# safijari/yag-slam

Hardware: AMD Instinct MI355X
Metric: pose hypotheses/sec (higher is better)
Workload: dtype u8

## Files before the change

yag_slam_amd/csrc/ym_abi_debug.hpp:

```cpp
int ym_debug_grid_info(ym_matcher *m, int item, ym_grid_info *info) {
    if (!m || !info) return set_err(YM_ERR_INVALID, "null argument");
    if (!m->last_valid || item < 0 || item >= m->last_B) return set_err(YM_ERR_INVALID, "no such item in the last call");
    const YmGeom &g = m->last_geom;
    info->width = g.win_w; info->height = g.win_w; info->pitch = g.pitch;
    info->origin_x = g.win_origin; info->origin_y = g.win_origin;
    info->storage_w = g.storage_w; info->storage_h = g.storage_w;
    info->roi_x = g.border; info->roi_y = g.border; info->roi_w = g.roi_w; info->roi_h = g.roi_w;
    YmItemState s;
    DEV_GUARD(m->device);
    HIP_TRY(hipStreamSynchronize(m->stream));
    HIP_TRY(hipMemcpy(&s, m->states.p + item, sizeof s, hipMemcpyDeviceToHost));
    info->offset_x = s.off_x; info->offset_y = s.off_y;
    return YM_OK;
}

int ym_debug_grid(ym_matcher *m, int item, uint8_t *out, int64_t out_bytes) {
    if (!m || !out) return set_err(YM_ERR_INVALID, "null argument");
    if (!m->last_valid || item < 0 || item >= m->last_B) return set_err(YM_ERR_INVALID, "no such item in the last call");
    const int64_t need = (int64_t)m->last_geom.pitch * m->last_geom.win_w;
    if (out_bytes < need) return set_err(YM_ERR_INVALID, "grid buffer too small: need %lld bytes", (long long)need);
    DEV_GUARD(m->device);
    HIP_TRY(hipStreamSynchronize(m->stream));
    HIP_TRY(hipMemcpy(out, m->grid.p + (size_t)item * m->last_grid_stride, (size_t)need, hipMemcpyDeviceToHost));
    return YM_OK;
// ... 24 lines not shown
    *n = s.nq;
    if (cap < s.nq) return set_err(YM_ERR_INVALID, "buffer too small: need %d points", s.nq);
    if (s.nq > 0)
        HIP_TRY(hipMemcpy(out_xy, s.ql, sizeof(double2) * s.nq, hipMemcpyDeviceToHost));
    return YM_OK;
}

int ym_debug_cells(ym_matcher *m, int item, int32_t *out, int64_t out_count, int32_t *max_n) {
    if (!m || !max_n) return set_err(YM_ERR_INVALID, "null argument");
    if (!m->last_valid || item < 0 || item >= m->last_B) return set_err(YM_ERR_INVALID, "no such item in the last call");
    *max_n = m->last_max_n;
    const size_t per = (size_t)m->last_max_base * m->last_max_n;
    if (!out) return YM_OK;
    if ((size_t)out_count < per * 2) return set_err(YM_ERR_INVALID, "buffer too small: need %zu ints", per * 2);
    DEV_GUARD(m->device);
    HIP_TRY(hipStreamSynchronize(m->stream));
    HIP_TRY(hipMemcpy(out, m->cells.p + (size_t)item * per, sizeof(int2) * per, hipMemcpyDeviceToHost));
    return YM_OK;
}

int ym_debug_option(ym_matcher *m, int option, int value) {
    if (m) { m->cache_gen++; m->list_key_valid = false; }
    if (!m) return set_err(YM_ERR_INVALID, "null matcher");
    if (option == 0) return set_err(YM_ERR_INVALID, "debug option 0 (an experimental correlate form) no longer exists");
    else if (option == 2) m->full_raster = value;
    else if (option == 3) m->corr_u = value;
    else if (option == 4) m->corr_pad_lds = value;
    else if (option == 5) m->corr_chunks = value;
    else if (option == 6) m->finish_form = value;
    else if (option == 9) m->corr_cw = value;
    else if (option == 10) m->select_global = value;
    else if (option == 41) m->select_split_max = value;
    else if (option == 11) m->finish_threads = value;
    else if (option == 12) m->keep_sums = value;
    else if (option == 13) m->corr_dedup = value;
    else if (option == 14) m->corr_region = value;
    else if (option == 15) m->corr_region_na = m->corr_region_nw = value;
    else if (option == 23) m->poll_completion = value != 0;
    else if (option == 24) m->use_scan_structure = value != 0;
    else if (option == 25) m->chain_margin = value;
    else if (option == 26) m->prepare_threads = value;
    else if (option == 28) {
        if (value == 0) { m->lds_min_batch = 64; m->rg_min_batch = 48; }
        else m->lds_min_batch = m->rg_min_batch = std::max(8, value);
    }
    else if (option == 42) m->rg_min_batch = value == 0 ? 48 : std::max(8, value);
    else if (option == 29) m->overlap_lists = value != 0;
    else if (option == 31) m->staged_queries = value != 0;
    else if (option == 30) m->tile_h_forced = value == YM_TILE_H || value == YM_TILE_H_TALL ? value : 0;
    else if (option == 16) m->raster_gx = value;
    else if (option == 17) m->corr_region_parts = value;
    else if (option == 21) m->corr_fuse_score = value;
    else if (option == 45) { m->list_cache_on = value != 0; m->list_key_valid = false; }
    else if (option == 46) m->yag_fast = value < 0 ? 0 : value > 2 ? 1 : value;
    else if (option == 43) m->rg2_h = value;
    else if (option == 44) {
#ifndef YM_EXPERIMENTAL
        return set_err(YM_ERR_UNSUPPORTED, "correlate_region2_kernel is compiled only into builds made with -DYM_EXPERIMENTAL");
#endif
        m->rg2_min_batch = value > 0 ? value : 1 << 30;
    }
    else if (option == 32) {
#ifndef YM_EXPERIMENTAL
        if (value >= 2) return set_err(YM_ERR_UNSUPPORTED, "correlate form %d is compiled only into builds made with -DYM_EXPERIMENTAL", value);
#endif
        m->corr_region_form = value;
    }
    else if (option == 33) m->corr_region_dbg = value;
    else if (option == 34) m->corr_region_rsplit = value;
    else if (option == 35) {
#ifndef YM_EXPERIMENTAL
        return set_err(YM_ERR_UNSUPPORTED, "correlate_item_kernel is compiled only into builds made with -DYM_EXPERIMENTAL");
#endif
        m->item_min_batch = value;
    }
    else if (option == 36) m->raster_planes_only = value;
    else if (option == 37) m->raster_no_rowtab = value;
    else if (option == 38) m->corr_region_pad_lds = value;
    else if (option == 39) m->keep_planes = value;
    else if (option == 40) m->tile_list_min_batch = value;
    else if (option == 19) m->corr_region_cap = value;
    else if (option == 20) m->corr_region_lds = value;
    else if (option == 18) m->raster_hits_per_tile = value;
    else if (option == 7) {
        m->cache_off = value == 1;
        m->cache_entries.clear();
        m->cache_index.clear();
        m->cache_used = 0;
    }
    else if (option == 8) {
        m->cache_limit = (size_t)std::max(1, value) << 10;
        HIP_TRY(hipStreamSynchronize(m->stream));
        m->cache_entries.clear();
        m->cache_index.clear();
        m->cache_used = 0;
        m->cache_arena.release();
    }
    else return set_err(YM_ERR_INVALID, "unknown option %d", option);
    return YM_OK;
}

int ym_debug_stamps(ym_matcher *m, int enable, uint64_t *out, int32_t count) {
    if (!m) return set_err(YM_ERR_INVALID, "null matcher");
    DEV_GUARD(m->device);
    HIP_TRY(hipStreamSynchronize(m->stream));
    if (out && count > 0)
// ... 54 lines not shown
```

yag_slam_amd/csrc/ym_host_enqueue.hpp:

```cpp
void enqueue_prepare(ym_matcher *m, const CallPlan &P) {
    ym::PrepareArgs a;
    a.scans = P.d_scans; a.items = P.d_items; a.g = P.g; a.lat = P.lc; a.states = m->states.p; a.qlocal = m->qlocal.p;
    a.cells = m->cells.p; a.bbox = m->bbox.p; a.ctrig = m->ctrig.p; a.hypcell = m->hypcell.p; a.probs = P.probs;
    a.max_n = P.max_n; a.max_base = P.max_base; a.nt_stride = P.nt_stride; a.dim_stride = P.dim_stride; a.stamps = P.stamps;
    a.use_inline = P.inline_desc ? 1 : 0;
    a.pad0 = 0;
    std::memset(&a.inl, 0, sizeof a.inl);
    if (a.use_inline) {
        a.inl.item = P.hi[0];
        for (int i = 0; i < P.nscans; i++) a.inl.scans[i] = P.hs[i];
    }
    a.qnp = m->qnp.p; a.jobs = P.d_jobs; a.job_slot = P.d_job_slot;
    a.fault = nullptr; a.step = 0; a.pad1 = 0;
    for (int k = 0; k < 4; k++) a.cell_box[k] = P.cell_box[k];
    if (P.chain_step) { a.fault = m->seq_fault.p; a.step = P.chain_step; }
    a.tile_max_zero = P.use_tile_list ? m->tile_max.p : nullptr;
    const size_t lds = YM_PREP_LDS_BYTES(P.max_n);
    if (P.split_prepare) {
        if (P.n_jobs > 0) hipLaunchKernelGGL(ym::points_kernel, dim3(P.n_jobs), dim3(YM_POINTS_THREADS), lds, m->stream, a);
        hipLaunchKernelGGL(ym::cells_kernel, dim3(P.max_base + 1, P.B), dim3(256), 0, m->stream, a);
    } else {
        if (P.B == 1 && m->prepare_threads != 512)
            hipLaunchKernelGGL(ym::prepare_kernel<1024>, dim3(P.max_base + 2, P.B), dim3(1024), lds, m->stream, a);
        else
// ... 114 lines not shown
            a.search_t = m->cfg.coarse_search_angle_offset * 0.5; a.step_t = m->cfg.coarse_angle_resolution;
        } else {
            a.search_xy = g.res * 2; a.step_xy = g.res; a.search_t = 0.0349 * 0.5; a.step_t = 0.00349;
        }
        a.coarse_angle_res = m->cfg.coarse_angle_resolution;
        a.states = m->states.p; a.host_out = reinterpret_cast<YmItemState *>(slot.result.dp);
        a.qlocal = m->qlocal.p; a.axes = m->yaxes.p; a.rot = nullptr;
        a.sums = m->sums.p + m->sums_pass_offset[pass]; a.out = m->resp.p;
        a.grid = m->grid.p; a.grid_stride = P.grid_stride; a.vol_stride = P.yvol;
        a.max_n = P.max_n; a.maxd = P.ymaxd; a.maxt = P.ymaxt;
        hipLaunchKernelGGL(ym::yag_setup_kernel, dim3(1, P.B), dim3(256), 0, m->stream, a);
        if (pass == 0 && P.lc.nx > 0) {
            a.lat_nx = P.lc.nx; a.lat_ny = P.lc.ny; a.lat_nt = P.lc.nt; a.step_cells = P.sx;
            a.nt_stride = P.nt_stride; a.dim_stride = P.dim_stride; a.ctrig = m->ctrig.p; a.hypcell = m->hypcell.p;
            a.lsums = m->sums.p + (size_t)2 * P.B * P.yvol; a.lsums_stride = P.sums_c; a.counters = m->yag_counters.p;
            hipLaunchKernelGGL(ym::yag_lattice_kernel, dim3(P.B), dim3(256), 0, m->stream, a);
            int rc = enqueue_correlate(m, P);
            if (rc) return rc;
            enqueue_score(m, slot, P);
        }
        if (pass == 1 && m->yag_fast) {
            a.fine_rows = m->yag_fast;
            a.n_items = P.B;
            if (P.B >= 64) hipLaunchKernelGGL(ym::yag_fine_kernel<64>, dim3(8 * P.ymaxt * ((P.B + 7) / 8)), dim3(64), 0, m->stream, a);
            else hipLaunchKernelGGL(ym::yag_fine_kernel<256>, dim3(8 * P.ymaxt * ((P.B + 7) / 8)), dim3(256), 0, m->stream, a);
        }
        hipLaunchKernelGGL(ym::yag_score_kernel, dim3((P.ymaxd * P.ymaxd + 255) / 256, P.ymaxt, P.B), dim3(256), 0, m->stream, a);
        if (P.B >= 16) hipLaunchKernelGGL(ym::yag_reduce_kernel<256>, dim3(P.B), dim3(256), 0, m->stream, a);
        else hipLaunchKernelGGL(ym::yag_reduce_kernel<1024>, dim3(P.B), dim3(1024), 0, m->stream, a);
    }
    return YM_OK;
}

ym::RegionArgs region_args(ym_matcher *m, const CallPlan &P) {
    ym::RegionArgs r;
    r.g = P.g; r.lat = P.lc; r.grid = m->grid.p; r.planes = m->planes.p; r.grid_stride = P.grid_stride; r.ctrig = m->ctrig.p;
    r.hypcell = m->hypcell.p; r.states = m->states.p; r.qrep = P.d_qrep; r.entries = m->rg_entries.p; r.entries_stride = P.rg_entries_stride;
    r.starts = m->rg_starts.p; r.starts_stride = P.rg_starts_stride; r.partial = m->partial.p; r.partial_stride = P.partial_stride;
    r.rbox = m->rg_rbox.p; r.rbox_stride = (size_t)P.rg_nregions * P.rg_parts; r.nw = P.rg_nw; r.parts = P.rg_parts;
    r.nt_stride = P.nt_stride; r.dim_stride = P.dim_stride; r.nrx = P.rg_nrx; r.nry = P.rg_nry; r.ng = P.rg_ng; r.nbins = P.rg_nbins;
    r.force_irregular = (m->corr_region == 2 || m->corr_region == 3) ? m->corr_region - 1 : 0; r.pad = m->corr_region_dbg; r.stamps = P.stamps;
    r.fuse_score = P.fuse_score ? 1 : 0; r.resp = P.resp; r.sums_stride = P.sums_c; r.blockmax = m->blockmax.p;
    r.probs = P.probs; r.probs_stride = (size_t)P.lc.nx * P.lc.ny; r.n_blocks = P.score_blocks;
    r.rg_h = YM_RG_H; r.rg_cls = YM_RG_CLS; r.rg_zero = YM_RG_ZERO; r.pad2 = 0;
#ifdef YM_EXPERIMENTAL
    r.rg_h = P.rg_ws ? YM_WS_H : YM_RG_H; r.rg_cls = P.rg_ws ? YM_WS_CLS : P.rg_item ? YM_IT_CLS : YM_RG_CLS;
    r.rg_zero = P.rg_ws ? YM_WS_ZERO : P.rg_item ? YM_IT_ZERO : YM_RG_ZERO;
#endif
    if (P.rg2) { r.rg_h = P.rg2_h; r.rg_cls = YM_RG_PITCH * (P.rg2_h + 26); r.rg_zero = 4 * r.rg_cls; }
    r.pad2 = ((1 << 21) + r.rg_h - 1) / r.rg_h;
    r.rg_w = 0; r.rg_pitch = YM_RG_PITCH; r.nregions = P.rg_nregions; r.pad3 = 0;
    r.walk = m->rg_walk.p; r.nitems = P.B; r.rsplit = P.rg_rsplit; r.pad4 = 0;
    r.lnw = P.rg_lnw; r.lparts = P.rg_lparts; r.entries_pstride = P.rg_entries_pstride;
    r.gpx = std::max(1, std::min((2 * std::max(m->n_cus, 8) / 8) / std::max(1, P.rg_parts), (P.B + 7) / 8));
    return r;
}

int enqueue_region_lists(ym_matcher *m, const CallPlan &P, hipStream_t st) {
    const ym::RegionArgs r = region_args(m, P);
#ifdef YM_EXPERIMENTAL
    if (P.rg_lparts == 1 && P.rg_lnw == P.lc.nt && (P.rg_ws || P.rg2 || P.rg_item || P.rg_pool)) {
        const size_t bin_lds = YM_BIN_LDS_BYTES(P.rg_nbins, P.rg_entries_stride, P.rg_nregions * P.rg_parts);
        if (bin_lds > m->bin_lds_limit) {
            HIP_TRY(hipFuncSetAttribute(reinterpret_cast<const void *>(ym::bin_whole_kernel<false>), hipFuncAttributeMaxDynamicSharedMemorySize, (int)bin_lds));
            m->bin_lds_limit = bin_lds;
        }
        hipLaunchKernelGGL(ym::bin_whole_kernel<false>, dim3(P.n_qslots), dim3(YM_BIN_THREADS), bin_lds, st, r);
        if (P.rg_ws) hipLaunchKernelGGL(ym::region_walk_kernel, dim3(P.rg_parts, P.n_qslots), dim3(64), 0, st, r);
        return YM_OK;
    }
#endif
    const size_t bin_lds = YM_BINP_LDS_BYTES(P.rg_nbins, P.rg_entries_pstride, P.rg_nregions);
    if (bin_lds > m->binp_lds_limit) {
#define YM_BINP_ATTR(Y, M) HIP_TRY(hipFuncSetAttribute(reinterpret_cast<const void *>(ym::bin_kernel<Y, M>), hipFuncAttributeMaxDynamicSharedMemorySize, (int)bin_lds))
        YM_BINP_ATTR(false, 18); YM_BINP_ATTR(false, 32); YM_BINP_ATTR(false, 64); YM_BINP_ATTR(true, 18); YM_BINP_ATTR(true, 32); YM_BINP_ATTR(true, 64);
#undef YM_BINP_ATTR
        m->binp_lds_limit = bin_lds;
    }
    const int per_thread = (P.rg_lnw * P.max_n + YM_BINP_THREADS - 1) / YM_BINP_THREADS;
    const dim3 bgrid(P.rg_lparts, P.n_qslots);
#define YM_BINP_LAUNCH(Y, M) hipLaunchKernelGGL((ym::bin_kernel<Y, M>), bgrid, dim3(YM_BINP_THREADS), bin_lds, st, r)
    if (P.yag) { if (per_thread <= 18) YM_BINP_LAUNCH(true, 18); else if (per_thread <= 32) YM_BINP_LAUNCH(true, 32); else YM_BINP_LAUNCH(true, 64); }
    else { if (per_thread <= 18) YM_BINP_LAUNCH(false, 18); else if (per_thread <= 32) YM_BINP_LAUNCH(false, 32); else YM_BINP_LAUNCH(false, 64); }
#undef YM_BINP_LAUNCH
    return YM_OK;
}

int enqueue_region_lists_aside(ym_matcher *m, CallPlan &P) {
    if (!m->side_stream) {
        HIP_TRY(hipStreamCreateWithFlags(&m->side_stream, hipStreamNonBlocking));
        pool_register_stream(m->device, m->side_stream, true);
        HIP_TRY(hipEventCreateWithFlags(&m->ev_fork, hipEventDisableTiming));
        HIP_TRY(hipEventCreateWithFlags(&m->ev_join, hipEventDisableTiming));
    }
    HIP_TRY(hipEventRecord(m->ev_fork, m->stream));
    return YM_OK;
}
int enqueue_region_lists_joined(ym_matcher *m, CallPlan &P) {
    HIP_TRY(hipStreamWaitEvent(m->side_stream, m->ev_fork, 0));
    int rc = enqueue_region_lists(m, P, m->side_stream);
    if (rc) return rc;
    HIP_TRY(hipEventRecord(m->ev_join, m->side_stream));
    P.lists_on_side_stream = true;
    return YM_OK;
}

// ... 211 lines not shown
```

yag_slam_amd/csrc/ym_host_matcher.hpp:

```cpp
struct ym_map {
    int device;
    int width, height;
    double *d_cgrid;
    uint8_t *d_g8;
};

struct ym_occupancy {
    int device;
    ym_occupancy_info info;
    std::vector<uint8_t> image;
};

struct ym_batch {
    std::vector<const ym_scan *> queries;
    std::vector<int32_t> item_query;
    std::vector<const ym_scan *> scans;
    std::vector<int32_t> offsets;
    mutable std::vector<int> cache_hints;
    mutable std::vector<int> query_hints;
    uint64_t uid = 0;
};

struct ym_matcher {
    ym_config cfg;
// ... 10 lines not shown
    int tall_tiles_min_window = 768;
    YmGeom geom;
    std::vector<uint8_t> kernel;
    std::vector<double> kernel_f;
    DevBuf<double> kernel_f_dev;
    DevBuf<double2> map_pts;
    int z2max = 0;
    DevBuf<uint8_t> ktab;
    DevBuf<uint8_t> rowtab;
    int n_rowtab = 0, rowtab_shift = -1;
    DevBuf<unsigned char> desc_dev;
    DevBuf<YmItemState> states;
    DevBuf<double2> qlocal;
    DevBuf<int32_t> qnp;
    DevBuf<unsigned char> tmp_cache;
    DevBuf<int2> cells;
    DevBuf<int4> bbox;
    DevBuf<uint8_t> grid;
    DevBuf<uint8_t> planes;
    DevBuf<uint8_t> tile_zero;
    DevBuf<uint8_t> sub_zero;
    size_t tz_sig[6] = {0, 0, 0, 0, 0, 0};
    std::vector<std::array<int, 4>> item_dirty;
    int tz_covered = 0;
    std::vector<unsigned char> planes_stale;
    DevBuf<double2> ctrig;
    DevBuf<int32_t> foffsets;
    DevBuf<int32_t> hypcell;
    DevBuf<uint16_t> partial;
    DevBuf<uint16_t> rg_entries;
    DevBuf<int32_t> rg_starts;
    DevBuf<uint32_t> rg_rbox;
    DevBuf<uint32_t> rg_walk;
    int n_cus = 0;
    size_t bin_lds_limit = 64 * 1024;
    size_t binp_lds_limit = 64 * 1024;
    int chain_margin = 1;
    uint64_t cache_gen = 1;
    int64_t seq_segments = 0, seq_faults = 0, seq_sync_steps = 0;
    int lds_min_batch = 64;
    int rg_min_batch = 48;
    int prepare_threads = 0;
    int last_wh = 0;
    bool use_scan_structure = true;
    bool poll_completion = true;
    int corr_region_nw = 0;
    int item_min_batch = 1 << 30;
    bool item_lds_set = false;
    int raster_planes_only = 0;
    int raster_no_rowtab = 0;
    int corr_region_rsplit = 0;
    int tile_list_min_batch = 48;
    int keep_planes = 0;
    int corr_region_pad_lds = 0;
    int corr_region_dbg = 0;
    int corr_region_form = 0;
    struct ListKey {
        uint64_t qid; double pose[3]; YmGeom g; YmLattice lc;
        int32_t nw, parts, nrx, nry, rg_h, force, nregions, ng; size_t es, ss; const void *pe, *ps, *pb;
    };
    ListKey list_key;
    bool list_key_valid = false, list_cache_on = true;
    int64_t list_cache_hits = 0;
    int rg2_min_batch = 1 << 30;
    int rg2_h = 128;
    size_t rg2_lds_limit = 0;
    int corr_fuse_score = 0;
    DevBuf<uint32_t> ga_units;
    DevBuf<int32_t> ga_starts;
    DevBuf<int32_t> ga_work;
    DevBuf<uint32_t> ga_counters;
    DevBuf<uint32_t> ga_lane_job;
    std::vector<uint32_t> ga_lane_job_host;
    size_t ga_lds_limit = 64 * 1024;
    DevBuf<uint32_t> sums;
    DevBuf<double> resp;
    DevBuf<double> blockmax;
    DevBuf<double> probs;
    int yag_fast = 1;
    int last_corr_form = -1;
    DevBuf<unsigned long long> yag_counters;
    DevBuf<double> yaxes;
    DevBuf<double2> yrot;
    DevBuf<double> seq_pose;
    DevBuf<int32_t> seq_fault;
    PinnedBuf seq_results;
    DevBuf<unsigned long long> stamps;
    bool stamps_on = false;
    int corr_u = 0;
    int full_raster = 0;
    struct CacheEntry { uint64_t id; size_t off; int n; double pose[3]; uint64_t stale_in_call; };
    uint64_t call_counter = 0;
    std::vector<CacheEntry> cache_entries;
    std::unordered_map<uint64_t, int> cache_index;
    DevBuf<unsigned char> cache_arena;
    size_t cache_used = 0;
    size_t cache_limit = (size_t)16 << 30;
    int cache_off = 0;
    int64_t cache_hits = 0, cache_misses = 0;
    DevBuf<unsigned> sel_scratch;
    DevBuf<unsigned> sel_tables;
    DevBuf<uint4> sel_rec;
    DevBuf<unsigned> sel_slot;
    DevBuf<uint32_t> tile_list;
    DevBuf<int32_t> tile_count;
    DevBuf<int32_t> tile_max;
// ... 31 lines not shown
```

yag_slam_amd/csrc/ym_k_region.hpp:

```cpp
#pragma once

namespace ym {

#ifndef YM_RG_PROF
#define YM_RG_PROF 0
#endif
#if YM_RG_PROF
#if YM_RG_PROF == 2
#define YM_RG_PH(i) do { if ((i) == 7 || (i) == 8 || (i) == 1 || (i) == 2 || (i) == 5) { const uint32_t t_ = (uint32_t)__builtin_amdgcn_s_memtime(); \
    if ((i) != 5) ph[(i) == 7 ? 0 : (i) == 8 ? 1 : (i) == 1 ? 2 : 3] += t_ - pt; pt = t_; } } while (0)
#else
#define YM_RG_PH(i) do { const uint32_t t_ = (uint32_t)__builtin_amdgcn_s_memtime(); if ((i) >= 2 && (i) <= 5) ph[(i) - 2] += t_ - pt; pt = t_; } while (0)
#endif
#else
#define YM_RG_PH(i) do { } while (0)
#endif

#ifndef YM_RG_ABLATE
#define YM_RG_ABLATE 0
#endif
#ifndef YM_RG_PRIO
#define YM_RG_PRIO 0
#endif
#define YM_RG_W 64
// ... 10 lines not shown
#define YM_RG_PLANES_SLACK(half_pitch) ((size_t)(2 * YM_RG_ROWS + 2 * YM_RG_H + 2) * (size_t)(half_pitch) + 256)
#define YM_RG_WINDOW_SLACK(pitch) ((size_t)(2 * YM_RG_ROWS + 2 * YM_RG_H + 2) * (size_t)(pitch) + 512)
static_assert(2 * YM_RG_ROWS + 2 * YM_RG_H + 2 >= 2 * (YM_RG_H - 1 + YM_RG_ROWS - 1) + 1 + 1, "YM_RG_PLANES_SLACK does not cover the rows a staged region reads");
static_assert(256 >= 16 * YM_RG_SEGS, "YM_RG_PLANES_SLACK does not cover the bytes a staged row reads");
static_assert(16 * YM_RG_SEGS >= YM_RG_W + 2 * YM_RG_G + 3 && YM_RG_PITCH >= 16 * YM_RG_SEGS && (YM_RG_PITCH / 4) % 2 == 1,
              "a staged row must hold the region, the patch margin and the misalignment, at an odd number of dwords per row");
#define YM_RG_MAX_BINS 8192
#define YM_RG_MAX_REGIONS 96
#define YM_RG_MAX_ENTRIES 28672
#define YM_RG_FLUSH 652
#define YM_BIN_THREADS 1024
#ifndef YM_BIN_MIN_WAVES
#define YM_BIN_MIN_WAVES 8
#endif
#define YM_BIN_LDS_BYTES(nbins, entries, nboxes) ((size_t)(YM_BIN_THREADS / 64 + YM_MAX_COARSE_NT + YM_RG_MAX_BINS / 32 + 1) * 4 + (size_t)(nbins) * 8 + ((size_t)(entries) * 2 + 15) / 16 * 16 + (size_t)(nboxes) * 16)

struct RegionArgs {
    YmGeom g;
    YmLattice lat;
    const uint8_t *grid;
    const uint8_t *planes;
    size_t grid_stride;
    const double2 *ctrig;
    const int32_t *hypcell;
    const YmItemState *states;
    const int32_t *qrep;
    uint16_t *entries;
    size_t entries_stride;
    int32_t *starts;
    size_t starts_stride;
    uint32_t *rbox;
    size_t rbox_stride;
    int32_t nw, parts;
    uint16_t *partial;
    size_t partial_stride;
    int32_t nt_stride, dim_stride;
    int32_t nrx, nry, ng, nbins;
    int32_t force_irregular;
    int32_t fuse_score;
    double *resp;
    size_t sums_stride;
    double *blockmax;
    double *probs;
    size_t probs_stride;
    int32_t n_blocks, pad;
    int32_t rg_h, rg_cls, rg_zero, pad2;
    int32_t rg_w, rg_pitch, nregions, pad3;
    uint32_t *walk;
    int32_t nitems, gpx;
    int32_t rsplit, pad4;
    unsigned long long *stamps;
    int32_t lnw, lparts;
    size_t entries_pstride;
};
__device__ __forceinline__ const int32_t *rg_part_starts(const RegionArgs &a, int qslot, int p) {
    return a.starts + (size_t)qslot * a.starts_stride + (size_t)p * (a.nbins + 1);
}
__device__ __forceinline__ bool rg_part_listed(const RegionArgs &a, int qslot, int p) {
    return a.starts[(size_t)qslot * a.starts_stride + (size_t)a.lparts * (a.nbins + 1) + p] >= 0;
}

__device__ __forceinline__ bool region_entry(const RegionArgs &a, int2 cell, int cx0, int cy0, int k, int &bin, unsigned &entry, int &region,
                                             unsigned &er, unsigned &ex, int bin_nw = -1) {
    const int X = cx0 + cell.x, Y = cy0 + cell.y;
    if (X < 0 || Y < 0) return false;
    const unsigned xc = (unsigned)X >> 1, yc = (unsigned)Y >> 1;
    const unsigned cls = (unsigned)((X & 1) | ((Y & 1) << 1));
#ifdef YM_EXPERIMENTAL
    if (a.rg_w) {
        const unsigned rx = xc / (unsigned)a.rg_w, ry = yc / (unsigned)a.rg_h;
        if ((int)rx >= a.nrx || (int)ry >= a.nry) return false;
        region = (int)((ry * (unsigned)a.nrx + rx) * 4u + cls);
        bin = region * a.lat.nt + k;
        er = yc - ry * (unsigned)a.rg_h;
        ex = xc - rx * (unsigned)a.rg_w;
        entry = er * (unsigned)a.rg_pitch + ex;
        return true;
    }
#endif
    if (yc >= 4096u) return false;
    const unsigned rx = xc / (unsigned)YM_RG_W, ry = __umul24(yc, (unsigned)a.pad2) >> 21;
    if ((int)rx >= a.nrx || (int)ry >= a.nry) return false;
    region = (int)(__umul24(ry, (unsigned)a.nrx) + rx);
    bin = (int)__umul24((unsigned)region, (unsigned)(bin_nw < 0 ? a.lat.nt : bin_nw)) + k;
    er = yc - __umul24(ry, (unsigned)a.rg_h);
    ex = xc - rx * YM_RG_W;
    entry = __umul24(cls, (unsigned)a.rg_cls) + __umul24(er, (unsigned)YM_RG_PITCH) + ex;
    return true;
}

#define YM_BINP_THREADS 512
#define YM_BINP_LDS_BYTES(nbins, entries, nboxes) ((size_t)(YM_BINP_THREADS / 64 + 16 + YM_RG_MAX_BINS / 32 + 1) * 4 + (size_t)(nbins) * 8 + ((size_t)(entries) * 2 + 15) / 16 * 16 + (size_t)(nboxes) * 16)
template <bool YAG, int MAXP>
__global__ __launch_bounds__(YM_BINP_THREADS, MAXP <= 18 ? 4 : 2) void bin_kernel(RegionArgs a) {
    constexpr int NT = YM_BINP_THREADS;
    extern __shared__ __attribute__((aligned(16))) unsigned char bin_smem[];
    int *wave_tot = reinterpret_cast<int *>(bin_smem);
    int *angle_tot = wave_tot + NT / 64;
    unsigned *region_bits = reinterpret_cast<unsigned *>(angle_tot + 16);
    int *regions_used = reinterpret_cast<int *>(region_bits + YM_RG_MAX_BINS / 32);
    unsigned (*cnt)[2] = reinterpret_cast<unsigned (*)[2]>(regions_used + 1);
    unsigned short *ent = reinterpret_cast<unsigned short *>(cnt + a.nbins);
    const int nboxes = a.nregions;
    unsigned (*box)[4] = reinterpret_cast<unsigned (*)[4]>(bin_smem + ((reinterpret_cast<unsigned char *>(ent + a.entries_pstride) - bin_smem) + 15) / 16 * 16);
    const int part = blockIdx.x, qs = blockIdx.y, b = a.qrep[qs], tid = threadIdx.x, lane = tid & 63;
    const YmItemState &st = a.states[b];
// ... 132 lines not shown
#pragma unroll
    for (int q = 0; q < MAXP; q++) {
        if (key[q] == 0xffffffffu) continue;
        const unsigned bin = (key[q] >> 16) & 0x1fffu, e = key[q] & 0xffffu;
        const unsigned rank = key[q] >> 29 | ((rank_hi[q >> 2] >> (8 * (q & 3))) & 0xffu) << 3;
        const unsigned f = cnt[bin][(e >> 1) & 1u];
        ent[((e & 1u) ? f >> 16 : f & 0xffffu) + rank] = (unsigned short)e;
    }
    __syncthreads();
    uint32_t *out = reinterpret_cast<uint32_t *>(a.entries + (size_t)qs * a.entries_stride + pos0);
    const uint32_t *src = reinterpret_cast<const uint32_t *>(ent);
    for (int i2 = tid; i2 < (padded_total + 1) / 2; i2 += NT) out[i2] = src[i2];
}

typedef unsigned int rg_u32x2 __attribute__((ext_vector_type(2)));
__device__ __forceinline__ void rg_perm_pair(const rg_u32x2 &pa, const rg_u32x2 &qa, const rg_u32x2 &pb, const rg_u32x2 &qb, uint32_t rr,
                                             uint32_t (&e)[4], uint32_t (&o)[4]) {
    const uint32_t s0 = pa.x + pb.x, s1 = pa.y + pb.y, s2 = qa.x + qb.x, s3 = qa.y + qb.y;
    const uint32_t selE = rr * 0x00010001u + 0x0c020c00u, selO = selE + 0x00010001u;
    e[0] = __builtin_amdgcn_perm(s1, s0, selE); o[0] = __builtin_amdgcn_perm(s1, s0, selO);
    e[1] = __builtin_amdgcn_perm(s2, s1, selE); o[1] = __builtin_amdgcn_perm(s2, s1, selO);
    e[2] = __builtin_amdgcn_perm(s3, s2, selE); o[2] = __builtin_amdgcn_perm(s3, s2, selO);
    e[3] = __builtin_amdgcn_perm(0u, s3, selE);
    o[3] = 0u;
}
__device__ __forceinline__ void rg_gather4(uint32_t (&acc)[8], uint32_t lane_off, uint2 ee ) {
    const uint32_t ad0 = lane_off + (ee.x & 0xffffu), ad1 = lane_off + (ee.x >> 16), ad2 = lane_off + (ee.y & 0xffffu), ad3 = lane_off + (ee.y >> 16);
#if YM_RG_ABLATE & 1
    acc[0] += ad0 ^ ad1 ^ ad2 ^ ad3;
    return;
#endif
    rg_u32x2 p0, q0, p1, q1, p2, q2, p3, q3;
    asm volatile("ds_read2_b32 %0, %8 offset1:1\n\tds_read2_b32 %1, %8 offset0:2 offset1:3\n\t"
                 "ds_read2_b32 %2, %9 offset1:1\n\tds_read2_b32 %3, %9 offset0:2 offset1:3\n\t"
                 "ds_read2_b32 %4, %10 offset1:1\n\tds_read2_b32 %5, %10 offset0:2 offset1:3\n\t"
                 "ds_read2_b32 %6, %11 offset1:1\n\tds_read2_b32 %7, %11 offset0:2 offset1:3\n\t"
                 "s_waitcnt lgkmcnt(4)"
                 : "=&v"(p0), "=&v"(q0), "=&v"(p1), "=&v"(q1), "=&v"(p2), "=&v"(q2), "=&v"(p3), "=&v"(q3)
                 : "v"(ad0 & ~3u), "v"(ad1 & ~3u), "v"(ad2 & ~3u), "v"(ad3 & ~3u)
                 : "memory");
    uint32_t e[2][4], o[2][4];
    rg_perm_pair(p0, q0, p1, q1, ad0 & 3u, e[0], o[0]);
    asm volatile("s_waitcnt lgkmcnt(0)" : "+v"(p2), "+v"(q2), "+v"(p3), "+v"(q3) : : "memory");
    rg_perm_pair(p2, q2, p3, q3, ad2 & 3u, e[1], o[1]);
#pragma unroll
    for (int j = 0; j < 4; j++) {
        acc[2 * j] = acc[2 * j] + e[0][j] + e[1][j];
        if (j < 3) acc[2 * j + 1] = acc[2 * j + 1] + o[0][j] + o[1][j];
    }
}

__device__ __forceinline__ void rg_odd(uint32_t (&)[8]) {}

template <int NW, bool WIN = false>
__global__ __launch_bounds__(64 * NW, NW <= 8 ? (3 * NW + 3) / 4 : 1 ) void correlate_region_kernel(RegionArgs a) {
    constexpr int NT = 64 * NW;
    constexpr int PER = (YM_RG_ROWS + (NT / 4) / YM_RG_SEGS - 1) / ((NT / 4) / YM_RG_SEGS);
    __shared__ __attribute__((aligned(16))) unsigned char region[YM_RG_LDS_BYTES];
    __shared__ int rlist[YM_RG_MAX_REGIONS];
    __shared__ uint32_t rboxl[YM_RG_MAX_REGIONS];
    __shared__ unsigned short seginfo[NW][YM_RG_MAX_REGIONS][2];
    __shared__ int rcount;
    int p;
    const int b = xcd_item_of_block_2d(p);
    const int rsplit = a.rsplit > 1 ? a.rsplit : 1, rsi = p / a.parts;
    p -= rsi * a.parts;
    const int tid = threadIdx.x, lane = tid & 63, wave = __builtin_amdgcn_readfirstlane(tid >> 6);
    const YmItemState &st = a.states[b];
    const int nt = a.lat.nt, nx = a.lat.nx, ny = a.lat.ny, ng = a.ng;
    const int k = p * NW + wave;
    const bool kvalid = k < nt;
    const int row = lane & 31, half = lane >> 5;
    const bool job = row < ny && half * YM_RG_G < nx;
    const int half_pitch = a.g.pitch / 2;
    const int plane_bytes = half_pitch * a.g.win_w;
    const uint8_t *__restrict__ planes = a.planes + (size_t)b * a.grid_stride;
    const int32_t *__restrict__ starts = rg_part_starts(a, st.qslot, p);
    const uint16_t *__restrict__ entries = a.entries + (size_t)st.qslot * a.entries_stride;
    const uint32_t lds0 = (uint32_t)(size_t)region;
    const uint32_t lane_off = lds0 + (uint32_t)((job ? row : 0) * YM_RG_PITCH + (half * YM_RG_G < nx ? half * YM_RG_G : 0));
    uint32_t acc[8];
#pragma unroll
    for (int j = 0; j < 8; j++) acc[j] = 0u;
    int in_set = 0, flushed = 0;
    auto flush = [&]() {
        if (flushed < ng) {
            rg_odd(acc);
            store_partial16(a.partial + (size_t)b * a.partial_stride + (((size_t)(rsi * ng + flushed) * nt + k) * 64 + lane) * 16, acc);
        }
#pragma unroll
        for (int j = 0; j < 8; j++) acc[j] = 0u;
        flushed++;
        in_set = 0;
    };
#if !YM_RG_PROF
    YM_STAMP(a, 8);
#endif
#if YM_RG_PROF
    uint32_t ph[4] = {0u, 0u, 0u, 0u};
    uint32_t pt = (uint32_t)__builtin_amdgcn_s_memtime();
    const uint32_t pt_begin = pt;
    const unsigned long long rt_begin = __builtin_amdgcn_s_memrealtime();
#endif
    const bool regular = st.regular[0] && a.force_irregular != 1 && rg_part_listed(a, st.qslot, p);
    if (regular) {
        const int k_lo = p * NW, k_hi = min(nt, k_lo + NW);
        const int nreg = a.nrx * a.nry;
        for (int i = tid; i < (YM_RG_LDS_BYTES - YM_RG_ZERO) / 4; i += NT) reinterpret_cast<uint32_t *>(region + YM_RG_ZERO)[i] = 0u;
        if (wave == 0) {
            int n = 0;
            for (int R0 = 0; R0 < nreg; R0 += 64) {
                const int R = R0 + lane;
                const bool has = R < nreg && starts[(size_t)R * NW] != starts[(size_t)R * NW + (k_hi - k_lo)];
                const unsigned long long mask = __ballot(has);
                const int at = n + __popcll(mask & ((1ull << lane) - 1ull));
                if (has && at % rsplit == rsi) rlist[at / rsplit] = R;
                n += __popcll(mask);
            }
            if (lane == 0) rcount = n > rsi ? (n - rsi + rsplit - 1) / rsplit : 0;
        }
        __syncthreads();
        const int nlist = rcount;
        {
            const uint32_t *rb = a.rbox + (size_t)st.qslot * a.rbox_stride;
            const uint32_t reach = (uint32_t)(nx > YM_RG_G ? 15 + YM_RG_G : 15);
            for (int i = tid; i < nlist; i += NT) {
                const uint32_t v = rb[(size_t)rlist[i] * a.parts + p];
                const uint32_t r0 = v & 0xffu, r1 = min((uint32_t)(YM_RG_ROWS - 1), ((v >> 8) & 0xffu) + (uint32_t)ny - 1u);
                const uint32_t s0 = ((v >> 16) & 0xfcu) >> 4, s1 = min((uint32_t)(YM_RG_SEGS - 1), ((v >> 24) + reach) >> 4);
                rboxl[i] = r0 | r1 << 8 | s0 << 16 | s1 << 24;
            }
        }
        if (kvalid)
            for (int i = lane; i < nlist; i += 64) {
                const int32_t *srow = starts + (size_t)rlist[i] * NW + wave;
                seginfo[wave][i][0] = (unsigned short)srow[0]; seginfo[wave][i][1] = (unsigned short)srow[1];
            }
        __syncthreads();
        constexpr int TPC = WIN ? NT / 2 : NT / 4;
        constexpr int NSEG = WIN ? 2 * YM_RG_SEGS : YM_RG_SEGS;
        constexpr int LPS = TPC / NSEG;
        constexpr int RSTEP = LPS;
        static_assert(LPS >= 1 && LPS * PER >= YM_RG_ROWS, "the copy tasks must cover a class image");
        const uint32_t cls = WIN ? 2u * ((uint32_t)tid / TPC) : (uint32_t)tid / TPC, j = (uint32_t)tid % TPC;
        const uint32_t seg = j % NSEG, r0 = j / NSEG;
        const bool copier = j < (uint32_t)(LPS * NSEG);
        const uint32_t src0 = WIN ? (2u * r0 + (cls >> 1)) * (uint32_t)a.g.pitch + 16u * seg
                                  : (cls & 1u) * (uint32_t)plane_bytes + (2u * r0 + (cls >> 1)) * (uint32_t)half_pitch + 16u * seg;
        const uint32_t src_step = WIN ? 2u * RSTEP * (uint32_t)a.g.pitch : 2u * RSTEP * (uint32_t)half_pitch;
        const uint32_t dst0 = (cls * YM_RG_ROWS + r0) * YM_RG_PITCH + (WIN ? 8u : 16u) * seg;
        uint4 v[PER];
        auto in_box = [&](int q, uint32_t bx, bool seg_in) {
            (void)q; (void)bx;
            return seg_in;
        };
        auto band_in = [&](int q, uint32_t bx) {
            return (uint32_t)(q * RSTEP) <= ((bx >> 8) & 0xffu) && (uint32_t)(q * RSTEP + RSTEP - 1) >= (bx & 0xffu);
        };
        const uint8_t *__restrict__ window = a.grid + (size_t)b * a.grid_stride;
        auto seg_inside = [&](uint32_t bx) {
            return WIN ? copier && seg >= 2u * ((bx >> 16) & 0xffu) && seg <= 2u * (bx >> 24) + 1u
                       : copier && seg >= ((bx >> 16) & 0xffu) && seg <= (bx >> 24);
        };
        auto stage_load = [&](int R, uint32_t bx) {
            const int RX = R % a.nrx, RY = R / a.nrx;
            const uint8_t *src = WIN ? window + ((size_t)(2 * RY * YM_RG_H) * a.g.pitch + (size_t)RX * (2 * YM_RG_W))
                                     : planes + ((size_t)(2 * RY * YM_RG_H) * half_pitch + (size_t)RX * YM_RG_W);
            const bool seg_in = seg_inside(bx);
#pragma unroll
            for (int q = 0; q < PER; q++)
#if YM_RG_ABLATE & 2
                v[q] = make_uint4((uint32_t)(size_t)src, seg_in, bx, q);
#else
                if (band_in(q, bx)) v[q] = *reinterpret_cast<const uint4 *>(src + (in_box(q, bx, seg_in) ? src0 + (uint32_t)q * src_step : 0u));
#endif
        };
        auto stage_store = [&](uint32_t bx) {
// ... 88 lines not shown
        }
    } else if (kvalid && job && rsi == 0) {
        const uint8_t *__restrict__ grid = a.grid + (size_t)b * a.grid_stride;
        const unsigned limit = (unsigned)(a.g.pitch * a.g.win_w);
        const int32_t *cx = a.hypcell + (size_t)b * 2 * a.dim_stride;
        const int32_t *cy = cx + a.dim_stride;
        const double2 cs = a.ctrig[(size_t)b * a.nt_stride + k];
        const double2 *ql = reinterpret_cast<const double2 *>(st.ql);
        const int nq = st.nq;
        const double add_x = a.g.semantics == 1 ? st.ylat[0] : st.off_x, add_y = a.g.semantics == 1 ? st.ylat[1] : st.off_y;
        for (int g = 0; g < ng; g++) {
            for (int j = 0; j < YM_RG_G; j++) {
                const int ix = half * YM_RG_G + j;
                if (ix >= nx) break;
                const int base = cy[row] * lin_pitch(a.g) + cx[ix];
                unsigned sum = 0;
                const int i1 = min(nq, (g + 1) * YM_RG_FLUSH);
                for (int i = g * YM_RG_FLUSH; i < i1; i++)
                    sum += cell_value(a.g, grid, limit, (unsigned)(base + lookup_offset_sem(a.g, ql[i], cs.x, cs.y, st.off_x, st.off_y, add_x, add_y, lin_pitch(a.g))));
                acc[2 * (j >> 2) + (j & 1)] += sum << (16 * ((j >> 1) & 1));
            }
            flush();
        }
    }
#if !YM_RG_PROF
    YM_STAMP(a, 9);
#endif
#if YM_RG_PROF
    auto prof_out = [&]() {
        if (a.stamps && lane == 0) {
            for (int i = 0; i < 4; i++) atomicAdd(a.stamps + 10 + i, (unsigned long long)ph[i]);
            atomicAdd(a.stamps + 8, (unsigned long long)(pt - pt_begin));
            atomicAdd(a.stamps + 9, __builtin_amdgcn_s_memrealtime() - rt_begin);
        }
    };
#endif
    if (!a.fuse_score) {
        if (!kvalid) return;
        while (flushed < ng) flush();
        return;
    }
    unsigned long long *pmax = reinterpret_cast<unsigned long long *>(region);
    const int nxy = nx * ny;
    double *dpen = reinterpret_cast<double *>(region) + ((nxy + 1) & ~1);
    __syncthreads();
    for (int i = tid; i < nxy; i += NT) {
        pmax[i] = 0ull;
        const int iy = i / nx, ix = i - iy * nx;
        const double x = -a.lat.off_x + ix * a.lat.step_x, y = -a.lat.off_y + iy * a.lat.step_y;
        dpen[i] = dist_penalty(a.g, x * x + y * y);
    }
    __syncthreads();
    if (kvalid) {
        unsigned tot[YM_RG_G];
        rg_odd(acc);
#pragma unroll
        for (int j = 0; j < YM_RG_G; j++) tot[j] = (acc[2 * (j >> 2) + (j & 1)] >> (16 * ((j >> 1) & 1))) & 0xffffu;
        for (int f = 0; f < min(flushed, ng); f++) {
            const uint16_t *pp = a.partial + (size_t)b * a.partial_stride + (((size_t)f * nt + k) * 64 + lane) * 16;
#pragma unroll
            for (int j = 0; j < YM_RG_G; j++) tot[j] += pp[j];
        }
        const double ct = st.center[2];
        const int nq = st.nq;
        const double angle = (ct - a.lat.angle_off) + k * a.lat.angle_res;
        const int ncb = (nxy + YM_SCORE_THREADS - 1) / YM_SCORE_THREADS;
        double bmax0 = -1.0, bmax1 = -1.0;
        const int c0 = row * nx + half * YM_RG_G, cb0 = job ? c0 / YM_SCORE_THREADS : 0;
#pragma unroll
        for (int j = 0; j < YM_RG_G; j++) {
            const int ix = half * YM_RG_G + j;
            if (job && ix < nx) {
                const int c = row * nx + ix;
                const double r = hyp_response_dp(a.g, a.lat.penalize, tot[j], nq, dpen[c], angle, ct);
                a.resp[(size_t)b * a.sums_stride + (size_t)k * nxy + c] = r;
                if (c / YM_SCORE_THREADS == cb0) bmax0 = r > bmax0 ? r : bmax0;
                else bmax1 = r > bmax1 ? r : bmax1;
                if (r > 0.0) atomicMax(&pmax[c], (unsigned long long)__double_as_longlong(r));
            }
        }
        for (int cb = 0; cb < ncb; cb++) {
            const double mine = !job ? -1.0 : cb == cb0 ? bmax0 : cb == cb0 + 1 ? bmax1 : -1.0;
            const double m = wave_reduce(mine, OpMaxD());
            if (lane == 0) a.blockmax[(size_t)b * a.n_blocks + (size_t)k * ncb + cb] = m;
        }
    }
    __syncthreads();
    for (int i = tid; i < nxy; i += NT)
        if (pmax[i]) atomicMax(reinterpret_cast<unsigned long long *>(a.probs) + (size_t)b * a.probs_stride + i, pmax[i]);
#if YM_RG_PROF
    YM_RG_PH(6);
    prof_out();
#endif
}


}
```

Measured before the change: 13.42 billion.

## Skip region-list entries whose grid footprint is entirely zero tiles

When building each block's region list, the correlate-region kernel now loads per-tile zero masks (tile_zero/sub_zero) into LDS. It drops regions whose bounding box covers only all-zero 8x8 sub-tiles, since those regions contribute nothing to the correlation sums. This is enabled only when a host-side signature check confirms the masks match the current grid, planes, pitch and tile height. The change also adds stamp counters for kept and dropped regions, a debug option to disable the pruning, and an asm barrier that recomputes row/half/job in the fused score epilogue, which likely affects register allocation. It adds an extra LDS fill and a __syncthreads per block, and it depends on the zero masks being current.

Measured after the change: 13.68 billion (median of 6 runs). 1.02x the previous value.

```diff
diff --git a/yag_slam_amd/csrc/ym_abi_debug.hpp b/yag_slam_amd/csrc/ym_abi_debug.hpp
--- a/yag_slam_amd/csrc/ym_abi_debug.hpp
+++ b/yag_slam_amd/csrc/ym_abi_debug.hpp
@@ -100,6 +100,7 @@
     else if (option == 17) m->corr_region_parts = value;
     else if (option == 21) m->corr_fuse_score = value;
     else if (option == 45) { m->list_cache_on = value != 0; m->list_key_valid = false; }
+    else if (option == 47) m->corr_region_list_all = value != 0;
     else if (option == 46) m->yag_fast = value < 0 ? 0 : value > 2 ? 1 : value;
     else if (option == 43) m->rg2_h = value;
     else if (option == 44) {
diff --git a/yag_slam_amd/csrc/ym_host_enqueue.hpp b/yag_slam_amd/csrc/ym_host_enqueue.hpp
--- a/yag_slam_amd/csrc/ym_host_enqueue.hpp
+++ b/yag_slam_amd/csrc/ym_host_enqueue.hpp
@@ -190,6 +190,16 @@
     r.rg_w = 0; r.rg_pitch = YM_RG_PITCH; r.nregions = P.rg_nregions; r.pad3 = 0;
     r.walk = m->rg_walk.p; r.nitems = P.B; r.rsplit = P.rg_rsplit; r.pad4 = 0;
     r.lnw = P.rg_lnw; r.lparts = P.rg_lparts; r.entries_pstride = P.rg_entries_pstride;
+    {
+        const size_t ntiles = (size_t)P.tiles_x * P.tiles_y;
+        const bool sig_ok = m->tz_sig[0] == (size_t)m->grid.p && m->tz_sig[1] == (size_t)m->planes.p && m->tz_sig[2] == P.grid_stride &&
+                            m->tz_sig[3] == (size_t)P.g.pitch && m->tz_sig[4] == (size_t)P.g.win_w && m->tz_sig[5] == (size_t)P.tile_h;
+        const bool known = sig_ok && m->tz_covered >= P.B && !m->corr_region_list_all && !m->raster_planes_only &&
+                           ntiles * 8 <= (size_t)YM_RG_ZERO && m->tile_zero.p && m->sub_zero.p;
+        r.tile_zero = known ? m->tile_zero.p : nullptr;
+        r.sub_zero = known ? m->sub_zero.p : nullptr;
+        r.tiles_x = P.tiles_x; r.tiles_y = P.tiles_y; r.tile_h = P.tile_h; r.pad5 = 0;
+    }
     r.gpx = std::max(1, std::min((2 * std::max(m->n_cus, 8) / 8) / std::max(1, P.rg_parts), (P.B + 7) / 8));
     return r;
 }
diff --git a/yag_slam_amd/csrc/ym_host_matcher.hpp b/yag_slam_amd/csrc/ym_host_matcher.hpp
--- a/yag_slam_amd/csrc/ym_host_matcher.hpp
+++ b/yag_slam_amd/csrc/ym_host_matcher.hpp
@@ -86,6 +86,7 @@
     int corr_region_rsplit = 0;
     int tile_list_min_batch = 48;
     int keep_planes = 0;
+    int corr_region_list_all = 0;
     int corr_region_pad_lds = 0;
     int corr_region_dbg = 0;
     int corr_region_form = 0;
diff --git a/yag_slam_amd/csrc/ym_k_region.hpp b/yag_slam_amd/csrc/ym_k_region.hpp
--- a/yag_slam_amd/csrc/ym_k_region.hpp
+++ b/yag_slam_amd/csrc/ym_k_region.hpp
@@ -86,6 +86,9 @@
     unsigned long long *stamps;
     int32_t lnw, lparts;
     size_t entries_pstride;
+    const uint8_t *tile_zero;
+    const uint8_t *sub_zero;
+    int32_t tiles_x, tiles_y, tile_h, pad5;
 };
 __device__ __forceinline__ const int32_t *rg_part_starts(const RegionArgs &a, int qslot, int p) {
     return a.starts + (size_t)qslot * a.starts_stride + (size_t)p * (a.nbins + 1);
@@ -324,6 +327,28 @@
 
 __device__ __forceinline__ void rg_odd(uint32_t (&)[8]) {}
 
+#define YM_RG_ZROWS 8
+__device__ __forceinline__ bool rg_tile_row_zero(const RegionArgs &a, const unsigned long long *zmask, int R, uint32_t v, int nx, int ny, int j) {
+    const int RY = R / a.nrx, RX = R - RY * a.nrx;
+    const int y0 = 2 * (RY * a.rg_h + (int)(v & 0xffu)), y1 = 2 * (RY * a.rg_h + (int)((v >> 8) & 0xffu) + ny - 1) + 1;
+    const int x0 = 2 * (RX * YM_RG_W + (int)((v >> 16) & 0xffu)), x1 = 2 * (RX * YM_RG_W + (int)(v >> 24) + nx - 1) + 1;
+    const int ths = a.tile_h == 64 ? 3 : 2;
+    const int sx0 = x0 >> 3, sx1 = x1 >> 3, sy0 = y0 >> 3, sy1 = y1 >> 3;
+    const int ty0 = sy0 >> ths, ty1 = sy1 >> ths, ty = ty0 + j;
+    if (x1 >= a.g.win_w || y1 >= a.g.win_w || x1 < x0 || y1 < y0 || ty1 - ty0 >= YM_RG_ZROWS) return false;
+    if (ty > ty1) return true;
+    const int b0 = max(sy0 - (ty << ths), 0), b1 = min(sy1 - (ty << ths), (1 << ths) - 1);
+    const unsigned long long rows = (b1 >= 7 ? ~0ull : (1ull << (8 * b1 + 8)) - 1ull) & ~((1ull << (8 * b0)) - 1ull);
+    bool zero = true;
+    for (int tx = sx0 >> 3; tx <= (sx1 >> 3); tx++) {
+        const int g0 = max(sx0 - 8 * tx, 0), g1 = min(sx1 - 8 * tx, 7);
+        const uint32_t cols = (((2u << g1) - 1u) & ~((1u << g0) - 1u)) * 0x01010101u;
+        const unsigned long long need = ((unsigned long long)cols | (unsigned long long)cols << 32) & rows;
+        zero = zero && (zmask[ty * a.tiles_x + tx] & need) == need;
+    }
+    return zero;
+}
+
 template <int NW, bool WIN = false>
 __global__ __launch_bounds__(64 * NW, NW <= 8 ? (3 * NW + 3) / 4 : 1 ) void correlate_region_kernel(RegionArgs a) {
     constexpr int NT = 64 * NW;
@@ -379,22 +404,57 @@
         const int k_lo = p * NW, k_hi = min(nt, k_lo + NW);
         const int nreg = a.nrx * a.nry;
         for (int i = tid; i < (YM_RG_LDS_BYTES - YM_RG_ZERO) / 4; i += NT) reinterpret_cast<uint32_t *>(region + YM_RG_ZERO)[i] = 0u;
+        const bool zknown = a.tile_zero != nullptr;
+        const uint32_t *rb = a.rbox + (size_t)st.qslot * a.rbox_stride;
+        bool has = false;
+        uint32_t hbox = 0u;
+        if (wave == 0 && lane < nreg) {
+            has = starts[(size_t)lane * NW] != starts[(size_t)lane * NW + (k_hi - k_lo)];
+            if (zknown) hbox = rb[(size_t)lane * a.parts + p];
+        }
+        if (zknown) {
+            const int ntiles = a.tiles_x * a.tiles_y;
+            const uint8_t *__restrict__ tz = a.tile_zero + (size_t)b * ntiles;
+            const uint2 *__restrict__ sz = reinterpret_cast<const uint2 *>(a.sub_zero) + (size_t)b * ntiles;
+            unsigned long long *zmask = reinterpret_cast<unsigned long long *>(region);
+            for (int i = tid; i < ntiles; i += NT) {
+                const uint2 s = sz[i];
+                zmask[i] = tz[i] ? ~0ull : ((unsigned long long)s.x | (unsigned long long)s.y << 32);
+            }
+            __syncthreads();
+        }
         if (wave == 0) {
-            int n = 0;
+            const unsigned long long *zmask = reinterpret_cast<const unsigned long long *>(region);
+            int n = 0, dropped = 0;
             for (int R0 = 0; R0 < nreg; R0 += 64) {
                 const int R = R0 + lane;
-                const bool has = R < nreg && starts[(size_t)R * NW] != starts[(size_t)R * NW + (k_hi - k_lo)];
-                const unsigned long long mask = __ballot(has);
+                if (R0 > 0) {
+                    has = R < nreg && starts[(size_t)R * NW] != starts[(size_t)R * NW + (k_hi - k_lo)];
+                    hbox = zknown && R < nreg ? rb[(size_t)R * a.parts + p] : 0u;
+                }
+                bool keep = has;
+                if (zknown && has) {
+                    bool zero = true;
+                    for (int j = 0; j < YM_RG_ZROWS && zero; j++) zero = rg_tile_row_zero(a, zmask, R, hbox, nx, ny, j);
+                    keep = !zero;
+                }
+                const unsigned long long mask = __ballot(keep);
                 const int at = n + __popcll(mask & ((1ull << lane) - 1ull));
-                if (has && at % rsplit == rsi) rlist[at / rsplit] = R;
+                if (keep && at % rsplit == rsi) rlist[at / rsplit] = R;
                 n += __popcll(mask);
-            }
-            if (lane == 0) rcount = n > rsi ? (n - rsi + rsplit - 1) / rsplit : 0;
+                dropped += __popcll(__ballot(has && !keep));
+            }
+            if (lane == 0) {
+                rcount = n > rsi ? (n - rsi + rsplit - 1) / rsplit : 0;
+                if (a.stamps) {
+                    atomicAdd(a.stamps + 20, (unsigned long long)rcount);
+                    if (rsi == 0) atomicAdd(a.stamps + 21, (unsigned long long)dropped);
+                }
+            }
         }
         __syncthreads();
         const int nlist = rcount;
         {
-            const uint32_t *rb = a.rbox + (size_t)st.qslot * a.rbox_stride;
             const uint32_t reach = (uint32_t)(nx > YM_RG_G ? 15 + YM_RG_G : 15);
             for (int i = tid; i < nlist; i += NT) {
                 const uint32_t v = rb[(size_t)rlist[i] * a.parts + p];
@@ -589,6 +649,10 @@
     }
     __syncthreads();
     if (kvalid) {
+        int tid_s = tid;
+        asm volatile("" : "+v"(tid_s));
+        const int row_s = tid_s & 31, half_s = (tid_s >> 5) & 1;
+        const bool job_s = row_s < ny && half_s * YM_RG_G < nx;
         unsigned tot[YM_RG_G];
         rg_odd(acc);
 #pragma unroll
@@ -603,12 +667,12 @@
         const double angle = (ct - a.lat.angle_off) + k * a.lat.angle_res;
         const int ncb = (nxy + YM_SCORE_THREADS - 1) / YM_SCORE_THREADS;
         double bmax0 = -1.0, bmax1 = -1.0;
-        const int c0 = row * nx + half * YM_RG_G, cb0 = job ? c0 / YM_SCORE_THREADS : 0;
+        const int c0 = row_s * nx + half_s * YM_RG_G, cb0 = job_s ? c0 / YM_SCORE_THREADS : 0;
 #pragma unroll
         for (int j = 0; j < YM_RG_G; j++) {
-            const int ix = half * YM_RG_G + j;
-            if (job && ix < nx) {
-                const int c = row * nx + ix;
+            const int ix = half_s * YM_RG_G + j;
+            if (job_s && ix < nx) {
+                const int c = row_s * nx + ix;
                 const double r = hyp_response_dp(a.g, a.lat.penalize, tot[j], nq, dpen[c], angle, ct);
                 a.resp[(size_t)b * a.sums_stride + (size_t)k * nxy + c] = r;
                 if (c / YM_SCORE_THREADS == cb0) bmax0 = r > bmax0 ? r : bmax0;
@@ -617,7 +681,7 @@
             }
         }
         for (int cb = 0; cb < ncb; cb++) {
-            const double mine = !job ? -1.0 : cb == cb0 ? bmax0 : cb == cb0 + 1 ? bmax1 : -1.0;
+            const double mine = !job_s ? -1.0 : cb == cb0 ? bmax0 : cb == cb0 + 1 ? bmax1 : -1.0;
             const double m = wave_reduce(mine, OpMaxD());
             if (lane == 0) a.blockmax[(size_t)b * a.n_blocks + (size_t)k * ncb + cb] = m;
         }
```
